# fallenshock/SinDDM

Measured on AMD Instinct MI355X. Metric: diffusion steps/sec (finest scale) + imgs/sec full multi-scale sample, 1/2/4/8 GPU, higher is better.
Workload: dtype f32 (3x3 convs: binary16 hi/lo split products -- Winograd-domain GEMMs with all 4 MFMA terms, fp32 accumulate; fp32-equivalent, error vs float64 = the fp32 oracle's: tests/test_gpu_h2.py; everything else fp32); 1 GPU; C3: 6-scale pyramid, T=1000, finest scale 411x512, batch 64 per GPU, dim=160; batch_per_gpu=64, global_batch=64, scale=5, parallelism=independent chains over 1 GPU(s), one all-gather of the images

## Files before the change

### include/sinddm_hip_debug.h

```cpp
#ifndef SINDDM_HIP_DEBUG_H
#define SINDDM_HIP_DEBUG_H

#include <stddef.h>
#include <stdint.h>

#ifdef __cplusplus
extern "C" {
#endif

int sinddm_prof_begin(void);
int sinddm_prof_end(double* conv_ms_total, int64_t* conv_launches, double* conv_flops_total);
int sinddm_prof_end2(double* conv_ms_total, int64_t* conv_launches, double* conv_flops_total,
                     double* conv_exec_flops_total);
int sinddm_prof_end3(int kind, double* ms_total, int64_t* launches, double* flops_total,
                     double* exec_flops_total, int reset);

int sinddm_debug_conv_path(int dim, int B, int H, int W);

int sinddm_debug_infer_path(int dim, int B, int H, int W);

int sinddm_debug_train_path(int dim, int B, int H, int W);

int sinddm_debug_block_train(const float* params, const float* packed, const float* packed_bwd, int dim, int l,
                             const float* x, const float* cond_bias, const float* grad_y, float* y, float* grad_x,
                             float* grad_params, float* dcond, int B, int H, int W, void* ws, size_t ws_bytes,
                             void* stream);

int sinddm_debug_wgrad_map(int Cin, int Cout, int64_t ntiles, int ncu, uint32_t* wg_out, int wg_cap, int32_t* splits_out,
                           int splits_cap);

#ifdef __cplusplus
}
#endif
#endif
```

### sinddm_amd/_lib.py

```python
from __future__ import annotations

import ctypes as C
import os
from typing import Optional

import torch

_HERE = os.path.dirname(os.path.abspath(__file__))
LIB_PATH = os.path.join(_HERE, "libsinddm_hip.so")

ABI_SYMBOLS = (
    "sinddm_abi_version", "sinddm_param_count", "sinddm_param_tensors", "sinddm_param_offset",
    "sinddm_packed_count", "sinddm_workspace_bytes", "sinddm_pack_weights", "sinddm_net_forward",
    "sinddm_q_sample", "sinddm_reverse_step", "sinddm_reverse_step_edit", "sinddm_upsample_bilinear", "sinddm_prof_begin", "sinddm_prof_end", "sinddm_prof_end2", "sinddm_prof_end3", "sinddm_debug_wgrad_map", "sinddm_debug_conv_path",
    "sinddm_debug_block_train", "sinddm_debug_infer_path", "sinddm_debug_train_path",
    "sinddm_train_workspace_bytes", "sinddm_packed_bwd_count", "sinddm_pack_weights_bwd",
    "sinddm_net_forward_train", "sinddm_net_backward", "sinddm_l1_loss_fwd_bwd", "sinddm_adam_ema_step",
    "sinddm_cond_embed", "sinddm_cond_stride", "sinddm_sample_chain", "sinddm_sample_chain2", "sinddm_sample_chain_ex",
    "sinddm_normal_fill", "sinddm_wrap_halo", "sinddm_upsample_bilinear_wrap", "sinddm_sample_chain_tile",
    "sinddm_sample_chain_keep", "sinddm_reverse_step_keep", "sinddm_normal_fill_samples", "sinddm_sample_chain_seeds",
)


ABI_VERSION = 3
DIM_FP32_CONVS = 0x10000
TILE_HALO = 16


class StepCoefs(C.Structure):
    _fields_ = [("mode", C.c_int), ("clip", C.c_int),
                ("sqrt_recip_ac_t", C.c_float), ("sqrt_recipm1_ac_t", C.c_float),
                ("coef1_t", C.c_float), ("coef2_t", C.c_float),
                ("gamma_t", C.c_float), ("gamma_tm1", C.c_float),
                ("sqrt_ac_tm1", C.c_float), ("sqrt_ac_t", C.c_float), ("sqrt_1m_ac_t", C.c_float),
                ("sqrt_1m_ac_tm1_mvar", C.c_float), ("sigma", C.c_float)]


class ChainOpts(C.Structure):
    _fields_ = [("edit_w", C.c_void_p), ("edit_c", C.c_void_p), ("noise", C.c_void_p)]


class KeepOpts(C.Structure):
    _fields_ = [("mask", C.c_void_p), ("x0", C.c_void_p), ("ab", C.POINTER(C.c_float))]
# ... 45 lines not shown
                                         i, i, i, i, p, sz, p, p, C.POINTER(C.c_int), C.POINTER(ChainOpts), i, i]),
        "sinddm_sample_chain_keep": (i, [p, p, p, p, p, p, C.POINTER(StepCoefs), C.POINTER(C.c_int), i, f, C.c_uint64, C.c_uint64,
                                         i, i, i, i, p, sz, p, p, C.POINTER(C.c_int), C.POINTER(ChainOpts), i, i,
                                         C.POINTER(KeepOpts)]),
        "sinddm_sample_chain_seeds": (i, [p, p, p, p, p, p, C.POINTER(StepCoefs), C.POINTER(C.c_int), i, f, C.c_uint64, C.c_uint64,
                                          i, i, i, i, p, sz, p, p, C.POINTER(C.c_int), C.POINTER(ChainOpts), i, i,
                                          C.POINTER(KeepOpts), p]),
        "sinddm_normal_fill_samples": (i, [p, i, i64, p, C.c_uint64, p]),
        "sinddm_reverse_step_keep": (i, [p, p, p, p, p, C.POINTER(StepCoefs), p, p, p, p, f, f, i, i, i, p]),
        "sinddm_wrap_halo": (i, [p, p, i, i, i, i, i, p]),
        "sinddm_upsample_bilinear_wrap": (i, [p, p, i, i, i, i, i, i, i, p]),
        "sinddm_normal_fill": (i, [p, i64, C.c_uint64, C.c_uint64, p]),
        "sinddm_upsample_bilinear": (i, [p, p, i, i, i, i, i, p]),
        "sinddm_prof_begin": (i, []),
        "sinddm_prof_end": (i, [C.POINTER(C.c_double), C.POINTER(C.c_int64), C.POINTER(C.c_double)]),
        "sinddm_prof_end2": (i, [C.POINTER(C.c_double), C.POINTER(C.c_int64), C.POINTER(C.c_double),
                                 C.POINTER(C.c_double)]),
        "sinddm_prof_end3": (i, [i, C.POINTER(C.c_double), C.POINTER(C.c_int64), C.POINTER(C.c_double),
                                 C.POINTER(C.c_double), i]),
        "sinddm_debug_wgrad_map": (i, [i, i, i64, i, C.POINTER(C.c_uint32), i, C.POINTER(C.c_int32), i]),
        "sinddm_debug_conv_path": (i, [i, i, i, i]),
        "sinddm_debug_infer_path": (i, [i, i, i, i]),
        "sinddm_debug_train_path": (i, [i, i, i, i]),
        "sinddm_debug_block_train": (i, [p, p, p, i, i, p, p, p, p, p, p, p, i, i, i, p, sz, p]),
        "sinddm_train_workspace_bytes": (sz, [i, i, i, i]),
        "sinddm_packed_bwd_count": (i64, [i]),
        "sinddm_pack_weights_bwd": (i, [p, p, i, p]),
        "sinddm_net_forward_train": (i, [p, p, p, p, i, f, p, i, i, i, i, p, sz, p]),
        "sinddm_net_backward": (i, [p, p, p, p, p, p, p, i, i, i, i, p, sz, p]),
        "sinddm_l1_loss_fwd_bwd": (i, [p, p, p, p, i64, f, p]),
        "sinddm_adam_ema_step": (i, [p, p, p, p, p, f, f, f, f, f, f, f, i, i64, p]),
    }
    for name, (res, args) in sig.items():
        if not hasattr(lib, name):
            continue
        fn = getattr(lib, name)
        fn.restype = res
        fn.argtypes = args
    _lib = lib
    return lib


def missing_symbols():
    lib = load()
    return [s for s in ABI_SYMBOLS if not hasattr(lib, s)]

# ... 20 lines not shown
```

### sinddm_amd/csrc/conv1x1.h

```cpp
#pragma once
#include "conv_mfma.h"

namespace sinddm {

constexpr int C1_THREADS = 256;
constexpr int C1_PIX = 256;
constexpr int C1_KC = 16;
constexpr int C1_PS = C1_PIX + 16;

template <int MT>
__global__ __launch_bounds__(C1_THREADS) void conv1x1_mfma_kernel(ConvArgs p, int tiles_per_img) {
    constexpr int CO_LDS = ConvCfg<MT, 4>::CO_LDS;
    constexpr int W_FLOATS = C1_KC * CO_LDS;
    constexpr int BUF = W_FLOATS + C1_KC * C1_PS;
    typedef __attribute__((address_space(3))) void* lds_ptr;
    extern __shared__ __attribute__((aligned(16))) float smem[];

    const int cb = blockIdx.y;
    const int tile = blockIdx.x;
    const int b = tile / tiles_per_img;
    const int p0 = (tile - b * tiles_per_img) * C1_PIX;
    const int tid = threadIdx.x, lane = tid & 63;
    const int wave = __builtin_amdgcn_readfirstlane(tid >> 6);
    const int l16 = lane & 15, kq = lane >> 4;
// ... 235 lines not shown
#pragma unroll
                    for (int j = 0; j < 4; ++j) v[j] = gelu_erf(v[j]);
                } else if constexpr (ACT == 2) {
#pragma unroll
                    for (int j = 0; j < 4; ++j) v[j] *= gelu_erf_grad(uv[mt & 1][r][j]);
                }
                if constexpr (RES) v += rv[mt & 1][r];
                if (C1B_ABL & 4) { if (v[0] + v[1] + v[2] + v[3] == 123.4f) p.out[tid] = v[1]; continue; }
                const unsigned o = off[mt & 1][r];
                __builtin_amdgcn_raw_buffer_store_b128(__builtin_bit_cast(u32x4, v), rs_out, (int)(straddle ? OOB : o), 0, 0);
                if (tail_tile && straddle) {
                    float* q = p.out + samp + (size_t)(co0 + mt * 16 + kq * 4 + r) * HW + px0;
#pragma unroll
                    for (int j = 0; j < 3; ++j)
                        if (j < keep) q[j] = v[j];
                }
            }
        }
        ctx = nctx;
    }
}

template <int MTT>
inline void conv1x1_all_launch(const ConvArgs& a, int tpi, int ntiles, hipStream_t st) {
    const size_t lds = ((size_t)((a.Cin2 + 15) / 16 * 4) * MTT * 64 + MTT * 16) * sizeof(float);
    const int cus = 256;
    const dim3 grid((unsigned)(ntiles < 2 * cus ? ntiles : 2 * cus), (unsigned)(a.Cout / (MTT * 16)));
#define C1B_GO(ACT, RES)                                                                                                \
    do {                                                                                                                \
        if ((a.H * a.W) % 4 == 0)                                                                                       \
            hipLaunchKernelGGL((conv1x1_all_kernel<MTT, ACT, 0, RES>), grid, dim3(C1_THREADS), lds, st, a, tpi, ntiles); \
        else                                                                                                            \
            hipLaunchKernelGGL((conv1x1_all_kernel<MTT, ACT, 1, RES>), grid, dim3(C1_THREADS), lds, st, a, tpi, ntiles); \
    } while (0)
    const int res = a.resid != nullptr;
    switch ((a.act & 0xff) * 2 + res) {
        case 0: C1B_GO(0, 0); break;
        case 1: C1B_GO(0, 1); break;
        case 2: C1B_GO(1, 0); break;
        case 3: C1B_GO(1, 1); break;
        case 4: C1B_GO(2, 0); break;
        default: C1B_GO(2, 1);
    }
#undef C1B_GO
}

#ifndef SINDDM_CONV1X1_V2
#define SINDDM_CONV1X1_V2 1
#endif
#ifndef SINDDM_CONV1X1_TAIL
#define SINDDM_CONV1X1_TAIL 1
#endif

inline int conv1x1_launch(const ConvArgs& a, int mt, hipStream_t st) {
    ConvProfiler& prof = conv_profiler();
    const bool rec = prof.on && prof.used < ConvProfiler::MAXREC;
    if (rec) {
        while (prof.created <= prof.used) {
            (void)hipEventCreate(&prof.ev[2 * prof.created]);
            (void)hipEventCreate(&prof.ev[2 * prof.created + 1]);
            ++prof.created;
        }
        (void)hipEventRecord(prof.ev[2 * prof.used], st);
    }
    const int HW = a.H * a.W;
    const int tpi = (HW + C1_PIX - 1) / C1_PIX;
    const dim3 grid((unsigned)(a.B * tpi), (unsigned)a.coblks);
    const int mtt = mt * a.coblks;
    if (SINDDM_CONV1X1_V2 && mt == 5 && (mtt == 5 || mtt == 10) && a.Cout == mtt * 16 && (SINDDM_CONV1X1_TAIL || HW % 4 == 0) && a.Cin2 <= 160) {
        const int ntiles = a.B * tpi;
        const size_t lds_all = ((size_t)((a.Cin2 + 15) / 16 * 4) * mtt * 64 + mtt * 16) * sizeof(float);
        if (ntiles >= 512 && mtt == 10 && lds_all <= 64 * 1024) conv1x1_all_launch<10>(a, tpi, ntiles, st);
        else if (ntiles >= 128) conv1x1_all_launch<5>(a, tpi, ntiles, st);
        else conv1x1_all_launch<1>(a, tpi, ntiles, st);
    } else
    switch (mt) {
        case 5: { constexpr size_t lds = 2 * (C1_KC * ConvCfg<5, 4>::CO_LDS + C1_KC * C1_PS) * sizeof(float);
                  hipLaunchKernelGGL(conv1x1_mfma_kernel<5>, grid, dim3(C1_THREADS), lds, st, a, tpi); break; }
        case 2: { constexpr size_t lds = 2 * (C1_KC * ConvCfg<2, 4>::CO_LDS + C1_KC * C1_PS) * sizeof(float);
                  hipLaunchKernelGGL(conv1x1_mfma_kernel<2>, grid, dim3(C1_THREADS), lds, st, a, tpi); break; }
        case 1: { constexpr size_t lds = 2 * (C1_KC * ConvCfg<1, 4>::CO_LDS + C1_KC * C1_PS) * sizeof(float);
                  hipLaunchKernelGGL(conv1x1_mfma_kernel<1>, grid, dim3(C1_THREADS), lds, st, a, tpi); break; }
        default: return SINDDM_E_BADSHAPE;
    }
    if (rec) {
        (void)hipEventRecord(prof.ev[2 * prof.used + 1], st);
        const double fl = 2.0 * a.B * a.H * a.W * (double)a.Cout * (double)a.Cin2;
        prof.note(2, fl, fl);
    }
    SINDDM_LAUNCH_CHECK();
    return 0;
}

}
```

### sinddm_amd/csrc/internal.h

```cpp
#pragma once
#include "common.h"

namespace sinddm {

struct PackSeg {
    long long dst;
    long long count;
    long long w;
    long long w2;
    int kind;
    int cin, cout, taps, nch, mt, co_lds;
    int transpose;
};
struct PackArgs {
    PackSeg seg[32];
    int nseg;
    long long total;
};
int pack_launch(const float* params, float* packed, const PackArgs& a, hipStream_t st);

struct TrainBufs {
    float* cond;
    float* emb;
    float* hpre;
    float* cvec;
    float* mvec;
    float* h[4];
    float* u[4];
    float* g[4];
    float* o[4];
    float* s[4];
    float* dcond;
    float* small;
    float* wscr;
    float* amax;
};

struct ChainStep;
int net_forward_impl(const NetPlan& P, const float* params, const float* packed, const float* x, const int64_t* t_dev,
                     int t_host, float scale, float* out, int B, int H, int W, void* ws, size_t ws_bytes,
                     hipStream_t st, const TrainBufs* tb, const ChainStep* cs = nullptr);

int block_forward(const NetPlan& P, int l, const float* params, const float* packed, const float* cur, const float* cond,
                  int cond_stride, float* hbuf, float* gbuf, float* obuf, float* upre, int B, int H, int W, hipStream_t st,
                  int Wt = 0, float* amax = nullptr);
int conv3x3_path(int cout, int cin, int coblks, int B, int H, int W);

struct ConvArgs;
bool wh_applies(const NetPlan& P, int B, int H, int W, int cin, int cout);
bool wh_enabled();
int wh_conv(const ConvArgs& c, hipStream_t st);
int wh_pack(const float* w, float* wsinv, void* img, int cin, int cout, int transpose, hipStream_t st);
int amax_tensor_launch(const float* x, float* amax, int B, long long per_sample, hipStream_t st);

int dwconv_launch(const float* x, const float* w, const float* bias, const float* cond, int cond_stride,
                  const float* addt, int flip, float* out, int B, int C, int H, int W, hipStream_t st, int pi = 0, int po = 0,
                  float* amax = nullptr);

}
```

### sinddm_amd/csrc/sinddm_fwd.hip

```cpp
#include "conv_mfma.h"
#include "conv_wino.h"
#include "conv_wino4.h"
#include "conv_wh.h"
#include "internal.h"
namespace sinddm {

ConvProfiler& conv_profiler() {
    static ConvProfiler p;
    return p;
}

__global__ void pack_kernel(const float* __restrict__ params, float* __restrict__ packed, PackArgs a) {
    long long i = (long long)blockIdx.x * blockDim.x + threadIdx.x;
    if (i >= a.total) return;
    int s = 0;
    long long base = 0;
    while (s < a.nseg - 1 && i >= base + a.seg[s].count) { base += a.seg[s].count; ++s; }
    const PackSeg& g = a.seg[s];
    const long long j = i - base;
    float v = 0.0f;
    if (g.kind == 0) {
        const int co_l = (int)(j % g.co_lds);
        long long r = j / g.co_lds;
        const int kc = (int)(r % KC); r /= KC;
// ... 347 lines not shown
        for (int h = 0; h < 2; ++h) {
            const int gx = x0 + lane + 64 * h;
            if (gx < po) {
#pragma unroll
                for (int r = 0; r < DW_RW; ++r) {
                    const int gy = y0 + wv * DW_RW + r;
                    if (gy < H) {
                        const size_t oidx = plane + (size_t)gy * po + gx;
                        const float ov = gx < W ? (addt ? o[r][h] + addt[oidx] : o[r][h]) : 0.0f;
                        mx = fmaxf(mx, fabsf(ov));
                        out[oidx] = ov;
                    }
                }
            }
        }
    }
    if (amax) amax_publish(mx, amax + (size_t)b * AMAX_STRIDE);
}

#ifndef DWR_ROWS_
#define DWR_ROWS_ 12
#endif
constexpr int DWR_ROWS = DWR_ROWS_;

__global__ __launch_bounds__(256) void dwconv5_rows_kernel(const float* __restrict__ x, const float* __restrict__ w,
                                                            const float* __restrict__ bias, const float* __restrict__ cond,
                                                            int cond_stride, const float* __restrict__ addt, int flip,
                                                            float* __restrict__ out, int C, int H, int W, int bandsX, int Wt,
                                                            float* __restrict__ amax) {
    const int c = blockIdx.y, b = blockIdx.z;
    const int by = blockIdx.x / bandsX, bx = blockIdx.x - by * bandsX;
    const int lane = threadIdx.x & 63, wv = threadIdx.x >> 6;
    const int x4 = (bx * 64 + lane) * 4;
    const int y0 = (by * 4 + wv) * DWR_ROWS;
    const size_t plane = ((size_t)b * C + c) * H * W;
    float wk[25];
#pragma unroll
    for (int k = 0; k < 25; ++k) wk[k] = w[c * 25 + (flip ? 24 - k : k)];
    const float add = (bias ? bias[c] : 0.0f) + (cond ? cond[(size_t)b * cond_stride + c] : 0.0f);
    if (y0 >= H) return;
    const __amdgpu_buffer_rsrc_t rsx = __builtin_amdgcn_make_buffer_rsrc(const_cast<float*>(x + plane), 0, H * W * 4, 0x00020000);
    constexpr int OOBI = 0x40000000;
    const bool colok = x4 < W;
    const bool lok = colok && x4 >= 4, rok = colok && x4 + 4 < W;
    f32x4 acc[DWR_ROWS];
#pragma unroll
    for (int r = 0; r < DWR_ROWS; ++r) acc[r] = f32x4{add, add, add, add};
#pragma unroll
    for (int ir = 0; ir < DWR_ROWS + 4; ++ir) {
        const int gy = y0 + ir - 2;
        const bool rowok = gy >= 0 && gy < H;
        const int base = (gy * W + x4) * 4;
        const f32x4 ql = __builtin_bit_cast(f32x4, __builtin_amdgcn_raw_buffer_load_b128(rsx, (rowok && lok) ? base - 16 : OOBI, 0, 0));
        const f32x4 qm = __builtin_bit_cast(f32x4, __builtin_amdgcn_raw_buffer_load_b128(rsx, (rowok && colok) ? base : OOBI, 0, 0));
        const f32x4 qr = __builtin_bit_cast(f32x4, __builtin_amdgcn_raw_buffer_load_b128(rsx, (rowok && rok) ? base + 16 : OOBI, 0, 0));
        const float in[8] = {ql[2], ql[3], qm[0], qm[1], qm[2], qm[3], qr[0], qr[1]};
#pragma unroll
        for (int r = 0; r < DWR_ROWS; ++r) {
            const int ky = ir - r;
            if (ky >= 0 && ky < 5) {
#pragma unroll
                for (int kx = 0; kx < 5; ++kx) {
#pragma unroll
                    for (int cc = 0; cc < 4; ++cc) acc[r][cc] = fmaf(wk[ky * 5 + kx], in[cc + kx], acc[r][cc]);
                }
            }
        }
    }
    float mx = 0.f;
#pragma unroll
    for (int r = 0; r < DWR_ROWS; ++r) {
        const int gy = y0 + r;
        if (colok && gy < H) {
            const size_t o = plane + (size_t)gy * W + x4;
            f32x4 v = acc[r];
            if (addt) v += *reinterpret_cast<const f32x4*>(addt + o);
            if (x4 + 4 > Wt) {
#pragma unroll
                for (int cc = 0; cc < 4; ++cc) v[cc] = x4 + cc < Wt ? v[cc] : 0.0f;
            }
            mx = fmaxf(fmaxf(mx, fmaxf(fabsf(v[0]), fabsf(v[1]))), fmaxf(fabsf(v[2]), fabsf(v[3])));
            *reinterpret_cast<f32x4*>(out + o) = v;
        }
    }
    if (amax) amax_publish(mx, amax + (size_t)b * AMAX_STRIDE);
}

#ifndef SINDDM_DW_ROWS
#define SINDDM_DW_ROWS 1
#endif

int dwconv_launch(const float* x, const float* w, const float* bias, const float* cond, int cond_stride,
                  const float* addt, int flip, float* out, int B, int C, int H, int W, hipStream_t st, int pi, int po,
                  float* amax) {
    if (pi <= 0) pi = W;
    if (po <= 0) po = W;
    if (SINDDM_DW_ROWS && pi % 4 == 0 && po == pi && pi >= 192) {
        const int bandsX = (pi + 255) / 256, bandsY = (H + 4 * DWR_ROWS - 1) / (4 * DWR_ROWS);
// ... 635 lines not shown
}
static size_t fwd_workspace_core(const NetPlan& P, int B, int H, int W) {
    const size_t act = align_up((size_t)B * P.dim * H * fwd_pitch(P, W) * sizeof(float), 256);
    return cond_region_bytes(P, B) + 4 * act + fwd_xpad_bytes(P, B, H, W);
}
static size_t fwd_workspace_bytes(const NetPlan& P, int B, int H, int W) {
    return fwd_workspace_core(P, B, H, W) + 2 * cond_region_bytes(P, (B + 1) / 2) + 4096;
}

struct ChainStep {
    const float* cond_row;
    const float* x_tilde;
    float* x_next;
    sinddm_step_coefs coefs;
    unsigned long long seed, stream_id;
    int b0;
    const float* edit_w;
    const float* edit_c;
    const float* noise;
    const float* keep_m;
    const float* keep_x0;
    float keep_a, keep_b;
    const unsigned long long* sseeds;
};

#define SINDDM_TAIL_LAUNCH(KERNEL, variant, grid, st, ...)                                                             \
    do {                                                                                                              \
        switch (variant) {                                                                                            \
            case 0: hipLaunchKernelGGL((KERNEL<false, false, false>), grid, dim3(256), 0, st, __VA_ARGS__); break;    \
            case 1: hipLaunchKernelGGL((KERNEL<true, false, false>), grid, dim3(256), 0, st, __VA_ARGS__); break;     \
            case 2: hipLaunchKernelGGL((KERNEL<false, true, false>), grid, dim3(256), 0, st, __VA_ARGS__); break;     \
            case 3: hipLaunchKernelGGL((KERNEL<true, true, false>), grid, dim3(256), 0, st, __VA_ARGS__); break;      \
            case 4: hipLaunchKernelGGL((KERNEL<false, false, true>), grid, dim3(256), 0, st, __VA_ARGS__); break;     \
            case 5: hipLaunchKernelGGL((KERNEL<true, false, true>), grid, dim3(256), 0, st, __VA_ARGS__); break;      \
            case 6: hipLaunchKernelGGL((KERNEL<false, true, true>), grid, dim3(256), 0, st, __VA_ARGS__); break;      \
            default: hipLaunchKernelGGL((KERNEL<true, true, true>), grid, dim3(256), 0, st, __VA_ARGS__); break;      \
        }                                                                                                             \
    } while (0)
static int tail_variant(const float* edit_w, const float* noise, const float* keep_m) {
    return (edit_w ? 1 : 0) | (noise ? 2 : 0) | (keep_m ? 4 : 0);
}

int conv3x3_path(int cout, int cin, int coblks, int B, int H, int W) {
    if (!wino_enabled() || cout % 4 != 0) return 0;
    const bool f24 = mt_for(cout) == 5 && cout % 80 == 0 && cin >= 16 && cin % 16 == 0;
    const bool v3 = SINDDM_WINO_V3 && f24 &&
                    (long long)B * ((W + 31) / 32) * ((H + 3) / 4) * coblks >= SINDDM_V3_MIN_ITEMS_PER_CU * wino2_cu_count();
    if (v3 && SINDDM_WINO_V4 && conv_wino4_applies(B, H, W, coblks)) return 4;
    return v3 ? 3 : 2;
}

int block_forward(const NetPlan& P, int l, const float* params, const float* packed, const float* cur, const float* cond,
                  int cond_stride, float* hbuf, float* gbuf, float* obuf, float* upre, int B, int H, int W, hipStream_t st,
                  int Wt, float* amax) {
    const BlockPlan& b = P.blk[l];
    const bool wha = amax && b.pk_q1 >= 0 && conv_wh_applies(P.fp32_convs, B, H, W, b.cin, b.cout);
    const bool whb = amax && b.pk_q2 >= 0 && conv_wh_applies(P.fp32_convs, B, H, W, b.cout, b.cout);
    int rc = Wt > 0 ? dwconv_launch(cur, params + b.dw_w, params + b.dw_b, cond, cond_stride, nullptr, 0, hbuf, B, b.cin, H,
                                    Wt, st, W, W, wha ? amax : nullptr)
                    : dwconv_launch(cur, params + b.dw_w, params + b.dw_b, cond, cond_stride, nullptr, 0, hbuf, B, b.cin, H,
                                    W, st, 0, 0, wha ? amax : nullptr);
    if (rc) return rc;
    const bool wino = wino_enabled();
    ConvArgs c1{};
    c1.in = hbuf; c1.bias = packed + b.pk_b1; c1.out = gbuf;
    c1.B = B; c1.H = H; c1.W = W; c1.Cin = b.cin; c1.Cout = b.cout; c1.nch1 = 0;
    c1.coblks = b.coblks; c1.act = 1; c1.zero = packed + P.pk_zero; c1.Wt = Wt;
    c1.out_pre = upre;
    constexpr int c3 = SINDDM_CONV_C3;
    const bool v3 = SINDDM_WINO_V3 && wino &&
                    (long long)B * ((W + 31) / 32) * ((H + 3) / 4) * b.coblks >= SINDDM_V3_MIN_ITEMS_PER_CU * wino2_cu_count();
    const bool v4 = SINDDM_WINO_V4 && v3 && conv_wino4_applies(B, H, W, b.coblks);
    if (wha) {
        c1.w3 = packed + b.pk_q1; c1.wsinv = packed + b.pk_qs1; c1.amax_in = amax; c1.amax_out = whb ? amax + 1 : nullptr;
        c1.bias = params + b.c1_b;
        rc = conv_wh_launch(c1, st);
    } else if (v3 && b.pk_w1f >= 0) {
        c1.w3 = packed + b.pk_w1f; c1.nch3 = b.nchw1;
        rc = v4 ? conv_wino4_launch(c1, st) : conv_wino3_launch(c1, st);
    } else if (wino && b.pk_wc1 >= 0 && b.cin % 4 == 0) {
        c1.w3 = packed + b.pk_wc1; c1.nch3 = b.nchw1;
        rc = conv_wino_launch(c1, b.mt, st);
    } else if (b.cin == 3 && c3) {
        const int nwg = ((H * W + 255) / 256) * B;
        int split = 1;
        while (split < 8 && nwg * split < 2048 && b.cout % (split * 2) == 0) split *= 2;
        hipLaunchKernelGGL(conv3x3_c3_gelu_kernel, dim3((H * W + 255) / 256, B, split), dim3(256), 0, st, hbuf,
                           params + b.c1_w, params + b.c1_b, gbuf, c1.out_pre, H, W, b.cout, b.cout / split, Wt > 0 ? Wt : W,
                           whb ? amax + 1 : nullptr);
        SINDDM_LAUNCH_CHECK();
        rc = 0;
    } else {
        c1.w3 = packed + b.pk_c1; c1.nch3 = b.nch1;
        rc = conv_launch(c1, b.mt, st);
    }
    if (rc) return rc;
    if (whb && !(wha || (b.cin == 3 && c3 && !(v3 && b.pk_w1f >= 0) && !(wino && b.pk_wc1 >= 0 && b.cin % 4 == 0)))) {
        rc = amax_tensor_launch(gbuf, amax + 1, B, (long long)b.cout * H * W, st);
        if (rc) return rc;
    }
    ConvArgs c2{};
    c2.in = gbuf; c2.out = obuf;
    c2.B = B; c2.H = H; c2.W = W; c2.Cin = b.cout; c2.Cout = b.cout;
    c2.coblks = b.coblks; c2.act = 0; c2.zero = packed + P.pk_zero; c2.Wt = Wt;
    if (wino && b.cout % 4 == 0) {
        if (b.nchr > 0) {
            ConvArgs r1{};
            r1.in2 = cur; r1.Cin2 = b.cin; r1.w1 = packed + b.pk_res; r1.nch1 = b.nchr; r1.nch3 = 0;
            r1.bias = packed + b.pk_b2; r1.out = obuf; r1.Cout = b.cout; r1.coblks = b.coblks;
            r1.B = B; r1.H = H; r1.W = W; r1.zero = packed + P.pk_zero;
            rc = conv1x1_launch(r1, b.mt, st);
            if (rc) return rc;
            c2.resid = obuf; c2.bias = nullptr;
        } else {
            c2.resid = cur; c2.bias = packed + b.pk_b2;
        }
        c2.nch1 = 0;
        if (whb) {
            c2.w3 = packed + b.pk_q2; c2.wsinv = packed + b.pk_qs2; c2.amax_in = amax + 1;
            rc = conv_wh_launch(c2, st);
        } else if (v3 && b.pk_w2f >= 0) {
            c2.w3 = packed + b.pk_w2f; c2.nch3 = b.nchw2;
            rc = v4 ? conv_wino4_launch(c2, st) : conv_wino3_launch(c2, st);
        } else {
            c2.w3 = packed + b.pk_wc2; c2.nch3 = b.nchw2;
            rc = conv_wino_launch(c2, b.mt, st);
        }
    } else {
        c2.w3 = packed + b.pk_c2; c2.bias = packed + b.pk_b2; c2.nch3 = b.nch2;
        if (b.nchr > 0) { c2.in2 = cur; c2.Cin2 = b.cin; c2.w1 = packed + b.pk_res; c2.nch1 = b.nchr; }
        else { c2.resid = cur; c2.nch1 = 0; }
        rc = conv_launch(c2, b.mt, st);
    }
    return rc;
}
// ... 76 lines not shown
        }
        if (!any) amax = nullptr;
        else if (hipMemsetAsync(amax, 0, (size_t)B * AMAX_STRIDE * sizeof(float), st) != hipSuccess) return SINDDM_E_BADARG;
    }
    const float* cur = x;
    if (padded) {
        const long long nrows = (long long)B * CHANNELS * H;
        const long long nq = nrows * (Wp / 4);
        hipLaunchKernelGGL(pad_rows_kernel, dim3((unsigned)((nq + 255) / 256)), dim3(256), 0, st, x, xpad, H, W, Wp, nrows);
        SINDDM_LAUNCH_CHECK();
        cur = xpad;
    }
    int freeb[4] = {0, 1, 2, 3};
    int curb = -1;
    for (int l = 0; l < 4; ++l) {
        const BlockPlan& b = P.blk[l];
        int sel[3], n = 0;
        for (int i = 0; i < 4 && n < 3; ++i)
            if (freeb[i] != curb) sel[n++] = freeb[i];
        float* hbuf = tb ? tb->h[l] : fb.buf[sel[0]];
        float* gbuf = tb ? tb->g[l] : fb.buf[sel[1]];
        float* obuf = tb ? tb->o[l] : fb.buf[sel[2]];
        const int rc = block_forward(P, l, params, packed, cur, fb.cond + b.cond_off, cond_stride, hbuf, gbuf, obuf,
                                     tb ? tb->u[l] : nullptr, B, H, Wp, st, padded ? W : 0, amax ? amax + 2 * l : nullptr);
        if (rc) return rc;
        cur = obuf;
        curb = sel[2];
    }
    const int HW = H * W;
    if (padded) {
        const unsigned gx = (unsigned)((H * (Wp / 4) + 255) / 256);
        if (cs && cs->x_next)
            SINDDM_TAIL_LAUNCH(final_conv_reverse_step_pitch_kernel, tail_variant(cs->edit_w, cs->noise, cs->keep_m), dim3(gx, B),
                               st, cur, params + P.fin_w, params + P.fin_b, x, cs->x_tilde, cs->x_next, cs->coefs, P.half, H, W,
                               Wp, cs->seed, cs->stream_id, cs->b0, cs->edit_w, cs->edit_c, cs->noise, cs->keep_m, cs->keep_x0,
                               cs->keep_a, cs->keep_b, cs->sseeds);
        else
            hipLaunchKernelGGL(final_conv1x1_pitch_kernel, dim3(gx, B), dim3(256), 0, st, cur, params + P.fin_w,
                               params + P.fin_b, out, P.half, H, W, Wp);
        SINDDM_LAUNCH_CHECK();
        return 0;
    }
    if (cs && cs->x_next && HW % 4 == 0) {
        SINDDM_TAIL_LAUNCH(final_conv_reverse_step_kernel, tail_variant(cs->edit_w, cs->noise, cs->keep_m),
                           dim3((HW / 4 + 255) / 256, B), st, cur, params + P.fin_w, params + P.fin_b, x, cs->x_tilde, cs->x_next,
                           cs->coefs, P.half, HW, cs->seed, cs->stream_id, cs->b0, cs->edit_w, cs->edit_c, cs->noise, cs->keep_m,
                           cs->keep_x0, cs->keep_a, cs->keep_b, cs->sseeds);
// ... 166 lines not shown
    NetPlan p = make_plan(dim);
    if (!p.ok) return SINDDM_E_BADSHAPE;
    hipStream_t st = static_cast<hipStream_t>(stream);
    hipStream_t sx = static_cast<hipStream_t>(aux_stream);
    const long long n = (long long)B * CHANNELS * H * W;
    long long bx = ((n + 3) / 4 + 255) / 256;
    if (bx > 8192) bx = 8192;
    if (ws_bytes < fwd_workspace_bytes(p, B, H, W)) return SINDDM_E_WORKSPACE;
    float* cond_tab = static_cast<float*>(ws);
    const bool fuse_tail = (H * W) % 4 == 0 || fwd_pitch(p, W) != W;
    const long long items = (long long)B * ((fwd_pitch(p, W) + 31) / 32) * ((H + 7) / 8) * 2;
    const long long ncu = wino2_cu_count();
    const long long rounds = (items + ncu - 1) / ncu;
    bool split = sx != nullptr && sx != st && B >= 2 && fuse_tail && n_steps > 0 && items < SINDDM_SPLIT_ITEMS_HI * ncu &&
                 items >= SINDDM_SPLIT_ITEMS_LO * ncu && (rounds * ncu - items) * 25 >= rounds * ncu;
    if (split && conv_wh_applies(p.fp32_convs, B, H, fwd_pitch(p, W), p.dim, p.dim))
        split = false;
    if (split && cond_region_bytes(p, B) + fwd_workspace_core(p, (B + 1) / 2, H, W) + fwd_workspace_core(p, B - (B + 1) / 2, H, W) > ws_bytes)
        split = false;
    const int Bh[2] = {split ? (B + 1) / 2 : B, split ? B - (B + 1) / 2 : 0};
    char* wsh[2] = {static_cast<char*>(ws), nullptr};
    size_t wsz[2] = {ws_bytes, 0};
    hipEvent_t ev_go = nullptr, ev_done = nullptr;
    if (split) {
        wsh[0] = static_cast<char*>(ws) + cond_region_bytes(p, B);
        wsz[0] = fwd_workspace_core(p, Bh[0], H, W);
        wsh[1] = wsh[0] + wsz[0];
        wsz[1] = fwd_workspace_core(p, Bh[1], H, W);
        if (hipEventCreateWithFlags(&ev_go, hipEventDisableTiming) != hipSuccess) return SINDDM_E_BADARG;
        if (hipEventCreateWithFlags(&ev_done, hipEventDisableTiming) != hipSuccess) {
            (void)hipEventDestroy(ev_go);
            return SINDDM_E_BADARG;
        }
    }
    const size_t hoff = (size_t)Bh[0] * CHANNELS * H * W;
    float* cur = x;
    float* nxt = x_alt;
    int rc = 0;
    if (tiled) rc = wrap_halo_launch(x, nullptr, B * CHANNELS, Hc, Wc, halo_y, halo_x, st);
    for (int i0 = 0; i0 < n_steps && rc == 0;) {
        int len = 1, dt = 0;
        if (i0 + 1 < n_steps) {
            dt = t_list[i0 + 1] - t_list[i0];
            len = 2;
            while (i0 + len < n_steps && len < CHAIN_COND_ROWS && t_list[i0 + len] - t_list[i0 + len - 1] == dt) ++len;
        }
// ... 4 lines not shown
        for (int l = 0; l < 4; ++l) {
            ca.mlp_w[l] = p.blk[l].mlp_w; ca.mlp_b[l] = p.blk[l].mlp_b;
            ca.tr_w[l] = p.blk[l].tr_w; ca.tr_b[l] = p.blk[l].tr_b;
            ca.cin[l] = p.blk[l].cin; ca.coff[l] = p.blk[l].cond_off;
        }
        hipLaunchKernelGGL(cond_kernel, dim3(len), dim3(128), 0, st, ca);
        if (hipGetLastError() != hipSuccess) { rc = SINDDM_E_BADARG; break; }
        if (split) {
            if (hipEventRecord(ev_go, st) != hipSuccess || hipStreamWaitEvent(sx, ev_go, 0) != hipSuccess) { rc = SINDDM_E_BADARG; break; }
        }
        for (int i = i0; i < i0 + len && rc == 0; ++i) {
            if (coefs[i].mode != 0 && !x_tilde) { rc = SINDDM_E_BADARG; break; }
            for (int h = 0; h < (split ? 2 : 1) && rc == 0; ++h) {
                const size_t o = h ? hoff : 0;
                ChainStep cs{};
                cs.cond_row = cond_tab + (size_t)(i - i0) * p.cond_stride;
                cs.x_tilde = x_tilde ? x_tilde + o : nullptr; cs.x_next = fuse_tail ? nxt + o : nullptr; cs.coefs = coefs[i];
                cs.seed = (unsigned long long)seed; cs.stream_id = (unsigned long long)(stream_id0 + (uint64_t)i);
                cs.b0 = h ? Bh[0] : 0;
                cs.edit_w = edit_w; cs.edit_c = edit_c; cs.noise = noise ? noise + (size_t)i * (size_t)n : nullptr;
                cs.keep_m = keep_m; cs.keep_x0 = keep_x0;
                if (keep_m) { cs.keep_a = keep_ab[2 * i]; cs.keep_b = keep_ab[2 * i + 1]; }
                cs.sseeds = sseeds ? sseeds + (h ? Bh[0] : 0) : nullptr;
                rc = net_forward_impl(p, params, packed, cur + o, nullptr, t_list[i], scale, eps + o, Bh[h], H, W, wsh[h], wsz[h],
                                      h ? sx : st, nullptr, &cs);
                if (tiled && fuse_tail && rc == 0)
                    rc = wrap_halo_launch(nxt + o, nullptr, Bh[h] * CHANNELS, Hc, Wc, halo_y, halo_x, h ? sx : st);
            }
            if (rc) break;
            if (!fuse_tail && sseeds) {
                const int chw = CHANNELS * H * W;
                unsigned gx = (unsigned)(((chw + 3) / 4 + 255) / 256);
                if (gx > 8192) gx = 8192;
                const unsigned long long sid = (unsigned long long)(stream_id0 + (uint64_t)i);
                const float ka = keep_m ? keep_ab[2 * i] : 1.0f, kb = keep_m ? keep_ab[2 * i + 1] : 0.0f;
#define SINDDM_SEEDED_TAIL(E, K)                                                                                          \
    hipLaunchKernelGGL((reverse_step_rng_samples_kernel<E, K>), dim3(gx, (unsigned)B), dim3(256), 0, st, cur, eps, x_tilde, nxt,  \
                       coefs[i], sid, sseeds, edit_w, edit_c, chw, H * W, keep_m, keep_x0, ka, kb)
                if (edit_w && keep_m) SINDDM_SEEDED_TAIL(true, true);
                else if (edit_w) SINDDM_SEEDED_TAIL(true, false);
                else if (keep_m) SINDDM_SEEDED_TAIL(false, true);
                else SINDDM_SEEDED_TAIL(false, false);
#undef SINDDM_SEEDED_TAIL
                if (hipGetLastError() != hipSuccess) { rc = SINDDM_E_BADARG; break; }
                if (tiled && (rc = wrap_halo_launch(nxt, nullptr, B * CHANNELS, Hc, Wc, halo_y, halo_x, st)) != 0) break;
            } else if (!fuse_tail) {
                SINDDM_TAIL_LAUNCH(reverse_step_rng_kernel, tail_variant(edit_w, noise, keep_m), dim3((unsigned)bx), st, cur, eps,
                                   x_tilde, nxt, coefs[i], n, (unsigned long long)seed,
                                   (unsigned long long)(stream_id0 + (uint64_t)i), edit_w, edit_c,
                                   noise ? noise + (size_t)i * (size_t)n : nullptr, CHANNELS * H * W, H * W, keep_m, keep_x0,
                                   keep_m ? keep_ab[2 * i] : 1.0f, keep_m ? keep_ab[2 * i + 1] : 0.0f);
                if (hipGetLastError() != hipSuccess) { rc = SINDDM_E_BADARG; break; }
                if (tiled && (rc = wrap_halo_launch(nxt, nullptr, B * CHANNELS, Hc, Wc, halo_y, halo_x, st)) != 0) break;
            }
            float* t_ = cur; cur = nxt; nxt = t_;
        }
        if (split) {
            if (hipEventRecord(ev_done, sx) != hipSuccess || hipStreamWaitEvent(st, ev_done, 0) != hipSuccess) {
                (void)hipStreamSynchronize(sx);
                if (!rc) rc = SINDDM_E_BADARG;
            }
        }
        i0 += len;
    }
    if (split) {
        (void)hipEventDestroy(ev_go);
        (void)hipEventDestroy(ev_done);
    }
    if (rc) return rc;
    if (result_in_alt) *result_in_alt = (cur == x_alt) ? 1 : 0;
    return 0;
}

int sinddm_sample_chain_ex(const float* params, const float* packed, float* x, float* x_alt, float* eps, const float* x_tilde,
                           const sinddm_step_coefs* coefs, const int* t_list, int n_steps, float scale, uint64_t seed,
                           uint64_t stream_id0, int dim, int B, int H, int W, void* ws, size_t ws_bytes, void* stream,
                           void* aux_stream, int* result_in_alt, const sinddm_chain_opts* opts) {
    return sample_chain_impl(params, packed, x, x_alt, eps, x_tilde, coefs, t_list, n_steps, scale, seed, stream_id0, dim, B, H, W,
                             ws, ws_bytes, stream, aux_stream, result_in_alt, opts, 0, 0, nullptr, nullptr);
}

int sinddm_sample_chain_tile(const float* params, const float* packed, float* x, float* x_alt, float* eps, const float* x_tilde,
                             const sinddm_step_coefs* coefs, const int* t_list, int n_steps, float scale, uint64_t seed,
                             uint64_t stream_id0, int dim, int B, int H, int W, void* ws, size_t ws_bytes, void* stream,
                             void* aux_stream, int* result_in_alt, const sinddm_chain_opts* opts, int halo_y, int halo_x) {
    return sinddm_sample_chain_keep(params, packed, x, x_alt, eps, x_tilde, coefs, t_list, n_steps, scale, seed, stream_id0, dim, B,
                                    H, W, ws, ws_bytes, stream, aux_stream, result_in_alt, opts, halo_y, halo_x, nullptr);
}

int sinddm_sample_chain_keep(const float* params, const float* packed, float* x, float* x_alt, float* eps, const float* x_tilde,
                             const sinddm_step_coefs* coefs, const int* t_list, int n_steps, float scale, uint64_t seed,
// ... 109 lines not shown
    p.flops = 0.0;
    p.exec_flops = 0.0;
    return 0;
}

int sinddm_prof_end(double* conv_ms_total, int64_t* conv_launches, double* conv_flops_total) {
    return sinddm_prof_end2(conv_ms_total, conv_launches, conv_flops_total, nullptr);
}

int sinddm_prof_end2(double* conv_ms_total, int64_t* conv_launches, double* conv_flops_total,
                     double* conv_exec_flops_total) {
    return sinddm_prof_end3(0, conv_ms_total, conv_launches, conv_flops_total, conv_exec_flops_total, 1);
}

int sinddm_debug_infer_path(int dim, int B, int H, int W) {
    NetPlan p = make_plan(dim);
    if (!p.ok || B <= 0 || H <= 0 || W <= 0) return SINDDM_E_BADARG;
    const BlockPlan& b = p.blk[2];
    const int Wp = fwd_pitch(p, W);
    if (b.pk_q2 >= 0 && conv_wh_applies(p.fp32_convs, B, H, Wp, b.cout, b.cout)) return 8;
    return conv3x3_path(b.cout, b.cout, b.coblks, B, H, Wp);
}

int sinddm_prof_end3(int kind, double* ms_total, int64_t* launches, double* flops_total, double* exec_flops_total,
                     int reset) {
    ConvProfiler& p = conv_profiler();
    p.on = false;
    double ms = 0.0, fl = 0.0, ex = 0.0;
    int64_t n = 0;
    for (int i = 0; i < p.used; ++i) {
        if (kind >= 10 ? (p.kind[i] != kind / 10 || p.gen[i] != kind % 10) : (kind != 0 && p.kind[i] != kind)) continue;
        hipError_t e = hipEventSynchronize(p.ev[2 * i + 1]);
        if (e != hipSuccess) return (int)e;
        float t = 0.f;
        e = hipEventElapsedTime(&t, p.ev[2 * i], p.ev[2 * i + 1]);
        if (e != hipSuccess) return (int)e;
        ms += t; fl += p.rec_flops[i]; ex += p.rec_exec[i]; ++n;
    }
    if (ms_total) *ms_total = ms;
    if (launches) *launches = n;
    if (flops_total) *flops_total = fl;
    if (exec_flops_total) *exec_flops_total = ex;
    if (reset) { p.used = 0; p.flops = 0.0; p.exec_flops = 0.0; }
    return 0;
}

// ... 31 lines not shown
```

Baseline: 721.2 sample-steps/s (finest scale, batch x steps/s, all GPUs).

## Overlap residual 1x1 projection on side stream; prefetch rows in depthwise conv

Each block's residual 1x1 projection now forks onto an auxiliary stream, gated by events, so it runs alongside the depthwise conv and first 3x3 conv on the main stream, using a reduced workgroups-per-CU grid. The 5x5 depthwise row kernel is restructured with a rolling register prefetch of input rows, narrower 64-bit edge loads, packed fp32x2 FMAs and a 4-waves occupancy bound. A debug entry point for the dwconv kernel is also added. The stream fork adds event overhead per block and the concurrent kernels compete for CUs, while the prefetch raises register pressure.

```diff
diff --git a/include/sinddm_hip_debug.h b/include/sinddm_hip_debug.h
--- a/include/sinddm_hip_debug.h
+++ b/include/sinddm_hip_debug.h
@@ -26,6 +26,10 @@
                              float* grad_params, float* dcond, int B, int H, int W, void* ws, size_t ws_bytes,
                              void* stream);
 
+int sinddm_debug_dwconv(const float* x, const float* w, const float* bias, const float* cond, int cond_stride,
+                        const float* addt, int flip, float* out, int B, int C, int H, int W, int Wt, float* amax,
+                        void* stream);
+
 int sinddm_debug_wgrad_map(int Cin, int Cout, int64_t ntiles, int ncu, uint32_t* wg_out, int wg_cap, int32_t* splits_out,
                            int splits_cap);
 
diff --git a/sinddm_amd/_lib.py b/sinddm_amd/_lib.py
--- a/sinddm_amd/_lib.py
+++ b/sinddm_amd/_lib.py
@@ -19,6 +19,7 @@
     "sinddm_cond_embed", "sinddm_cond_stride", "sinddm_sample_chain", "sinddm_sample_chain2", "sinddm_sample_chain_ex",
     "sinddm_normal_fill", "sinddm_wrap_halo", "sinddm_upsample_bilinear_wrap", "sinddm_sample_chain_tile",
     "sinddm_sample_chain_keep", "sinddm_reverse_step_keep", "sinddm_normal_fill_samples", "sinddm_sample_chain_seeds",
+    "sinddm_debug_dwconv",
 )
 
 
@@ -110,6 +111,7 @@
         "sinddm_debug_conv_path": (i, [i, i, i, i]),
         "sinddm_debug_infer_path": (i, [i, i, i, i]),
         "sinddm_debug_train_path": (i, [i, i, i, i]),
+        "sinddm_debug_dwconv": (i, [p, p, p, p, i, p, i, p, i, i, i, i, i, p, p]),
         "sinddm_debug_block_train": (i, [p, p, p, i, i, p, p, p, p, p, p, p, i, i, i, p, sz, p]),
         "sinddm_train_workspace_bytes": (sz, [i, i, i, i]),
         "sinddm_packed_bwd_count": (i64, [i]),
diff --git a/sinddm_amd/csrc/conv1x1.h b/sinddm_amd/csrc/conv1x1.h
--- a/sinddm_amd/csrc/conv1x1.h
+++ b/sinddm_amd/csrc/conv1x1.h
@@ -281,10 +281,10 @@
 }
 
 template <int MTT>
-inline void conv1x1_all_launch(const ConvArgs& a, int tpi, int ntiles, hipStream_t st) {
+inline void conv1x1_all_launch(const ConvArgs& a, int tpi, int ntiles, hipStream_t st, int wg_per_cu) {
     const size_t lds = ((size_t)((a.Cin2 + 15) / 16 * 4) * MTT * 64 + MTT * 16) * sizeof(float);
     const int cus = 256;
-    const dim3 grid((unsigned)(ntiles < 2 * cus ? ntiles : 2 * cus), (unsigned)(a.Cout / (MTT * 16)));
+    const dim3 grid((unsigned)(ntiles < wg_per_cu * cus ? ntiles : wg_per_cu * cus), (unsigned)(a.Cout / (MTT * 16)));
 #define C1B_GO(ACT, RES)                                                                                                \
     do {                                                                                                                \
         if ((a.H * a.W) % 4 == 0)                                                                                       \
@@ -311,7 +311,7 @@
 #define SINDDM_CONV1X1_TAIL 1
 #endif
 
-inline int conv1x1_launch(const ConvArgs& a, int mt, hipStream_t st) {
+inline int conv1x1_launch(const ConvArgs& a, int mt, hipStream_t st, int wg_per_cu = 2) {
     ConvProfiler& prof = conv_profiler();
     const bool rec = prof.on && prof.used < ConvProfiler::MAXREC;
     if (rec) {
@@ -329,9 +329,9 @@
     if (SINDDM_CONV1X1_V2 && mt == 5 && (mtt == 5 || mtt == 10) && a.Cout == mtt * 16 && (SINDDM_CONV1X1_TAIL || HW % 4 == 0) && a.Cin2 <= 160) {
         const int ntiles = a.B * tpi;
         const size_t lds_all = ((size_t)((a.Cin2 + 15) / 16 * 4) * mtt * 64 + mtt * 16) * sizeof(float);
-        if (ntiles >= 512 && mtt == 10 && lds_all <= 64 * 1024) conv1x1_all_launch<10>(a, tpi, ntiles, st);
-        else if (ntiles >= 128) conv1x1_all_launch<5>(a, tpi, ntiles, st);
-        else conv1x1_all_launch<1>(a, tpi, ntiles, st);
+        if (ntiles >= 512 && mtt == 10 && lds_all <= 64 * 1024) conv1x1_all_launch<10>(a, tpi, ntiles, st, wg_per_cu);
+        else if (ntiles >= 128) conv1x1_all_launch<5>(a, tpi, ntiles, st, wg_per_cu);
+        else conv1x1_all_launch<1>(a, tpi, ntiles, st, wg_per_cu);
     } else
     switch (mt) {
         case 5: { constexpr size_t lds = 2 * (C1_KC * ConvCfg<5, 4>::CO_LDS + C1_KC * C1_PS) * sizeof(float);
diff --git a/sinddm_amd/csrc/internal.h b/sinddm_amd/csrc/internal.h
--- a/sinddm_amd/csrc/internal.h
+++ b/sinddm_amd/csrc/internal.h
@@ -37,13 +37,17 @@
 };
 
 struct ChainStep;
+struct SideStream {
+    hipStream_t sx;
+    hipEvent_t ev_fork, ev_join;
+};
 int net_forward_impl(const NetPlan& P, const float* params, const float* packed, const float* x, const int64_t* t_dev,
                      int t_host, float scale, float* out, int B, int H, int W, void* ws, size_t ws_bytes,
                      hipStream_t st, const TrainBufs* tb, const ChainStep* cs = nullptr);
 
 int block_forward(const NetPlan& P, int l, const float* params, const float* packed, const float* cur, const float* cond,
                   int cond_stride, float* hbuf, float* gbuf, float* obuf, float* upre, int B, int H, int W, hipStream_t st,
-                  int Wt = 0, float* amax = nullptr);
+                  int Wt = 0, float* amax = nullptr, const SideStream* side = nullptr);
 int conv3x3_path(int cout, int cin, int coblks, int B, int H, int W);
 
 struct ConvArgs;
diff --git a/sinddm_amd/csrc/sinddm_fwd.hip b/sinddm_amd/csrc/sinddm_fwd.hip
--- a/sinddm_amd/csrc/sinddm_fwd.hip
+++ b/sinddm_amd/csrc/sinddm_fwd.hip
@@ -393,15 +393,19 @@
 #define DWR_ROWS_ 12
 #endif
 constexpr int DWR_ROWS = DWR_ROWS_;
-
-__global__ __launch_bounds__(256) void dwconv5_rows_kernel(const float* __restrict__ x, const float* __restrict__ w,
+#ifndef DWR_PF_
+#define DWR_PF_ 6
+#endif
+constexpr int DWR_PF = DWR_PF_;
+
+__global__ __launch_bounds__(256, 4) void dwconv5_rows_kernel(const float* __restrict__ x, const float* __restrict__ w,
                                                             const float* __restrict__ bias, const float* __restrict__ cond,
                                                             int cond_stride, const float* __restrict__ addt, int flip,
                                                             float* __restrict__ out, int C, int H, int W, int bandsX, int Wt,
                                                             float* __restrict__ amax) {
     const int c = blockIdx.y, b = blockIdx.z;
     const int by = blockIdx.x / bandsX, bx = blockIdx.x - by * bandsX;
-    const int lane = threadIdx.x & 63, wv = threadIdx.x >> 6;
+    const int lane = threadIdx.x & 63, wv = __builtin_amdgcn_readfirstlane(threadIdx.x >> 6);
     const int x4 = (bx * 64 + lane) * 4;
     const int y0 = (by * 4 + wv) * DWR_ROWS;
     const size_t plane = ((size_t)b * C + c) * H * W;
@@ -413,30 +417,49 @@
     const __amdgpu_buffer_rsrc_t rsx = __builtin_amdgcn_make_buffer_rsrc(const_cast<float*>(x + plane), 0, H * W * 4, 0x00020000);
     constexpr int OOBI = 0x40000000;
     const bool colok = x4 < W;
-    const bool lok = colok && x4 >= 4, rok = colok && x4 + 4 < W;
-    f32x4 acc[DWR_ROWS];
-#pragma unroll
-    for (int r = 0; r < DWR_ROWS; ++r) acc[r] = f32x4{add, add, add, add};
+    const unsigned cl = (colok && x4 >= 4) ? x4 * 4 - 8 : OOBI;
+    const unsigned cm = colok ? x4 * 4 : OOBI;
+    const unsigned cr = (colok && x4 + 4 < W) ? x4 * 4 + 16 : OOBI;
+    f32x2 ql[DWR_PF], qr[DWR_PF];
+    f32x4 qm[DWR_PF];
+    auto load_row = [&](int ir) __attribute__((always_inline)) {
+        const int gy = y0 + ir - 2;
+        unsigned ro = (unsigned)gy < (unsigned)H ? (unsigned)(gy * W * 4) : (unsigned)OOBI;
+        asm volatile("" : "+s"(ro));
+        const int s = ir % DWR_PF;
+        ql[s] = __builtin_bit_cast(f32x2, __builtin_amdgcn_raw_buffer_load_b64(rsx, (int)(cl + ro), 0, 0));
+        qm[s] = __builtin_bit_cast(f32x4, __builtin_amdgcn_raw_buffer_load_b128(rsx, (int)(cm + ro), 0, 0));
+        qr[s] = __builtin_bit_cast(f32x2, __builtin_amdgcn_raw_buffer_load_b64(rsx, (int)(cr + ro), 0, 0));
+    };
+#pragma unroll
+    for (int ir = 0; ir < DWR_PF; ++ir) load_row(ir);
+    f32x2 acc[DWR_ROWS][2];
+#pragma unroll
+    for (int r = 0; r < DWR_ROWS; ++r) acc[r][0] = acc[r][1] = f32x2{add, add};
 #pragma unroll
     for (int ir = 0; ir < DWR_ROWS + 4; ++ir) {
-        const int gy = y0 + ir - 2;
-        const bool rowok = gy >= 0 && gy < H;
-        const int base = (gy * W + x4) * 4;
-        const f32x4 ql = __builtin_bit_cast(f32x4, __builtin_amdgcn_raw_buffer_load_b128(rsx, (rowok && lok) ? base - 16 : OOBI, 0, 0));
-        const f32x4 qm = __builtin_bit_cast(f32x4, __builtin_amdgcn_raw_buffer_load_b128(rsx, (rowok && colok) ? base : OOBI, 0, 0));
-        const f32x4 qr = __builtin_bit_cast(f32x4, __builtin_amdgcn_raw_buffer_load_b128(rsx, (rowok && rok) ? base + 16 : OOBI, 0, 0));
-        const float in[8] = {ql[2], ql[3], qm[0], qm[1], qm[2], qm[3], qr[0], qr[1]};
+        const int s = ir % DWR_PF;
+        const f32x2 ev[4] = {ql[s], f32x2{qm[s][0], qm[s][1]}, f32x2{qm[s][2], qm[s][3]}, qr[s]};
+        const f32x2 od[3] = {f32x2{ql[s][1], qm[s][0]}, f32x2{qm[s][1], qm[s][2]}, f32x2{qm[s][3], qr[s][0]}};
 #pragma unroll
         for (int r = 0; r < DWR_ROWS; ++r) {
             const int ky = ir - r;
             if (ky >= 0 && ky < 5) {
 #pragma unroll
                 for (int kx = 0; kx < 5; ++kx) {
-#pragma unroll
-                    for (int cc = 0; cc < 4; ++cc) acc[r][cc] = fmaf(wk[ky * 5 + kx], in[cc + kx], acc[r][cc]);
+                    const float wt = wk[ky * 5 + kx];
+                    const f32x2 w2{wt, wt};
+                    const f32x2 i0 = (kx & 1) ? od[kx >> 1] : ev[kx >> 1];
+                    const f32x2 i1 = (kx & 1) ? od[(kx >> 1) + 1] : ev[(kx >> 1) + 1];
+                    acc[r][0] = __builtin_elementwise_fma(w2, i0, acc[r][0]);
+                    acc[r][1] = __builtin_elementwise_fma(w2, i1, acc[r][1]);
                 }
             }
         }
+#pragma unroll
+        for (int r = 0; r < DWR_ROWS; ++r)
+            if (ir - r >= 0 && ir - r < 5) asm volatile("" : "+v"(acc[r][0]), "+v"(acc[r][1]));
+        if (ir + DWR_PF < DWR_ROWS + 4) load_row(ir + DWR_PF);
     }
     float mx = 0.f;
 #pragma unroll
@@ -444,7 +467,7 @@
         const int gy = y0 + r;
         if (colok && gy < H) {
             const size_t o = plane + (size_t)gy * W + x4;
-            f32x4 v = acc[r];
+            f32x4 v{acc[r][0][0], acc[r][0][1], acc[r][1][0], acc[r][1][1]};
             if (addt) v += *reinterpret_cast<const f32x4*>(addt + o);
             if (x4 + 4 > Wt) {
 #pragma unroll
@@ -1126,6 +1149,7 @@
     const float* keep_x0;
     float keep_a, keep_b;
     const unsigned long long* sseeds;
+    const SideStream* side;
 };
 
 #define SINDDM_TAIL_LAUNCH(KERNEL, variant, grid, st, ...)                                                             \
@@ -1154,12 +1178,20 @@
     return v3 ? 3 : 2;
 }
 
-int block_forward(const NetPlan& P, int l, const float* params, const float* packed, const float* cur, const float* cond,
-                  int cond_stride, float* hbuf, float* gbuf, float* obuf, float* upre, int B, int H, int W, hipStream_t st,
-                  int Wt, float* amax) {
+#ifndef SINDDM_SIDE_STREAM
+#define SINDDM_SIDE_STREAM 1
+#endif
+#ifndef SINDDM_SIDE_FIRST
+#define SINDDM_SIDE_FIRST 1
+#endif
+#ifndef SINDDM_SIDE_WG_PER_CU
+#define SINDDM_SIDE_WG_PER_CU 1
+#endif
+
+static int block_head(const NetPlan& P, int l, const float* params, const float* packed, const float* cur, const float* cond,
+                      int cond_stride, float* hbuf, float* gbuf, float* upre, int B, int H, int W, hipStream_t st, int Wt,
+                      float* amax, bool wha, bool whb) {
     const BlockPlan& b = P.blk[l];
-    const bool wha = amax && b.pk_q1 >= 0 && conv_wh_applies(P.fp32_convs, B, H, W, b.cin, b.cout);
-    const bool whb = amax && b.pk_q2 >= 0 && conv_wh_applies(P.fp32_convs, B, H, W, b.cout, b.cout);
     int rc = Wt > 0 ? dwconv_launch(cur, params + b.dw_w, params + b.dw_b, cond, cond_stride, nullptr, 0, hbuf, B, b.cin, H,
                                     Wt, st, W, W, wha ? amax : nullptr)
                     : dwconv_launch(cur, params + b.dw_w, params + b.dw_b, cond, cond_stride, nullptr, 0, hbuf, B, b.cin, H,
@@ -1203,18 +1235,51 @@
         rc = amax_tensor_launch(gbuf, amax + 1, B, (long long)b.cout * H * W, st);
         if (rc) return rc;
     }
+    return 0;
+}
+
+int block_forward(const NetPlan& P, int l, const float* params, const float* packed, const float* cur, const float* cond,
+                  int cond_stride, float* hbuf, float* gbuf, float* obuf, float* upre, int B, int H, int W, hipStream_t st,
+                  int Wt, float* amax, const SideStream* side) {
+    const BlockPlan& b = P.blk[l];
+    const bool wha = amax && b.pk_q1 >= 0 && conv_wh_applies(P.fp32_convs, B, H, W, b.cin, b.cout);
+    const bool whb = amax && b.pk_q2 >= 0 && conv_wh_applies(P.fp32_convs, B, H, W, b.cout, b.cout);
+    const bool wino = wino_enabled();
+    const bool proj = wino && b.cout % 4 == 0 && b.nchr > 0;
+    auto proj_launch = [&](hipStream_t s, int wg_per_cu) {
+        ConvArgs r1{};
+        r1.in2 = cur; r1.Cin2 = b.cin; r1.w1 = packed + b.pk_res; r1.nch1 = b.nchr; r1.nch3 = 0;
+        r1.bias = packed + b.pk_b2; r1.out = obuf; r1.Cout = b.cout; r1.coblks = b.coblks;
+        r1.B = B; r1.H = H; r1.W = W; r1.zero = packed + P.pk_zero;
+        return conv1x1_launch(r1, b.mt, s, wg_per_cu);
+    };
+    const bool fork = side != nullptr && whb && proj;
+    if (fork && (hipEventRecord(side->ev_fork, st) != hipSuccess || hipStreamWaitEvent(side->sx, side->ev_fork, 0) != hipSuccess))
+        return SINDDM_E_BADARG;
+    int rc = 0;
+    if (fork && SINDDM_SIDE_FIRST) rc = proj_launch(side->sx, SINDDM_SIDE_WG_PER_CU);
+    if (!rc) rc = block_head(P, l, params, packed, cur, cond, cond_stride, hbuf, gbuf, upre, B, H, W, st, Wt, amax, wha, whb);
+    if (fork && !SINDDM_SIDE_FIRST && !rc) rc = proj_launch(side->sx, SINDDM_SIDE_WG_PER_CU);
+    if (fork) {
+        if (hipEventRecord(side->ev_join, side->sx) != hipSuccess || hipStreamWaitEvent(st, side->ev_join, 0) != hipSuccess) {
+            (void)hipStreamSynchronize(side->sx);
+            if (!rc) rc = SINDDM_E_BADARG;
+        }
+    }
+    if (rc) return rc;
+    const bool v3 = SINDDM_WINO_V3 && wino &&
+                    (long long)B * ((W + 31) / 32) * ((H + 3) / 4) * b.coblks >= SINDDM_V3_MIN_ITEMS_PER_CU * wino2_cu_count();
+    const bool v4 = SINDDM_WINO_V4 && v3 && conv_wino4_applies(B, H, W, b.coblks);
     ConvArgs c2{};
     c2.in = gbuf; c2.out = obuf;
     c2.B = B; c2.H = H; c2.W = W; c2.Cin = b.cout; c2.Cout = b.cout;
     c2.coblks = b.coblks; c2.act = 0; c2.zero = packed + P.pk_zero; c2.Wt = Wt;
     if (wino && b.cout % 4 == 0) {
-        if (b.nchr > 0) {
-            ConvArgs r1{};
-            r1.in2 = cur; r1.Cin2 = b.cin; r1.w1 = packed + b.pk_res; r1.nch1 = b.nchr; r1.nch3 = 0;
-            r1.bias = packed + b.pk_b2; r1.out = obuf; r1.Cout = b.cout; r1.coblks = b.coblks;
-            r1.B = B; r1.H = H; r1.W = W; r1.zero = packed + P.pk_zero;
-            rc = conv1x1_launch(r1, b.mt, st);
-            if (rc) return rc;
+        if (proj) {
+            if (!fork) {
+                rc = proj_launch(st, 2);
+                if (rc) return rc;
+            }
             c2.resid = obuf; c2.bias = nullptr;
         } else {
             c2.resid = cur; c2.bias = packed + b.pk_b2;
@@ -1337,7 +1402,8 @@
         float* gbuf = tb ? tb->g[l] : fb.buf[sel[1]];
         float* obuf = tb ? tb->o[l] : fb.buf[sel[2]];
         const int rc = block_forward(P, l, params, packed, cur, fb.cond + b.cond_off, cond_stride, hbuf, gbuf, obuf,
-                                     tb ? tb->u[l] : nullptr, B, H, Wp, st, padded ? W : 0, amax ? amax + 2 * l : nullptr);
+                                     tb ? tb->u[l] : nullptr, B, H, Wp, st, padded ? W : 0, amax ? amax + 2 * l : nullptr,
+                                     cs ? cs->side : nullptr);
         if (rc) return rc;
         cur = obuf;
         curb = sel[2];
@@ -1550,6 +1616,16 @@
     char* wsh[2] = {static_cast<char*>(ws), nullptr};
     size_t wsz[2] = {ws_bytes, 0};
     hipEvent_t ev_go = nullptr, ev_done = nullptr;
+    SideStream side{sx, nullptr, nullptr};
+    const bool side_on = SINDDM_SIDE_STREAM && !split && sx != nullptr && sx != st && n_steps > 0 &&
+                         conv_wh_applies(p.fp32_convs, B, H, fwd_pitch(p, W), p.dim, p.dim);
+    if (side_on) {
+        if (hipEventCreateWithFlags(&side.ev_fork, hipEventDisableTiming) != hipSuccess) return SINDDM_E_BADARG;
+        if (hipEventCreateWithFlags(&side.ev_join, hipEventDisableTiming) != hipSuccess) {
+            (void)hipEventDestroy(side.ev_fork);
+            return SINDDM_E_BADARG;
+        }
+    }
     if (split) {
         wsh[0] = static_cast<char*>(ws) + cond_region_bytes(p, B);
         wsz[0] = fwd_workspace_core(p, Bh[0], H, W);
@@ -1600,6 +1676,7 @@
                 cs.keep_m = keep_m; cs.keep_x0 = keep_x0;
                 if (keep_m) { cs.keep_a = keep_ab[2 * i]; cs.keep_b = keep_ab[2 * i + 1]; }
                 cs.sseeds = sseeds ? sseeds + (h ? Bh[0] : 0) : nullptr;
+                cs.side = side_on ? &side : nullptr;
                 rc = net_forward_impl(p, params, packed, cur + o, nullptr, t_list[i], scale, eps + o, Bh[h], H, W, wsh[h], wsz[h],
                                       h ? sx : st, nullptr, &cs);
                 if (tiled && fuse_tail && rc == 0)
@@ -1645,6 +1722,10 @@
         (void)hipEventDestroy(ev_go);
         (void)hipEventDestroy(ev_done);
     }
+    if (side_on) {
+        (void)hipEventDestroy(side.ev_fork);
+        (void)hipEventDestroy(side.ev_join);
+    }
     if (rc) return rc;
     if (result_in_alt) *result_in_alt = (cur == x_alt) ? 1 : 0;
     return 0;
@@ -1800,6 +1881,15 @@
     return conv3x3_path(b.cout, b.cout, b.coblks, B, H, Wp);
 }
 
+int sinddm_debug_dwconv(const float* x, const float* w, const float* bias, const float* cond, int cond_stride,
+                        const float* addt, int flip, float* out, int B, int C, int H, int W, int Wt, float* amax, void* stream) {
+    if (!x || !w || !out || B <= 0 || C <= 0 || H <= 0 || W <= 0 || Wt < 0 || Wt > W) return SINDDM_E_BADARG;
+    if ((long long)H * W * 4 >= 0x40000000LL) return SINDDM_E_BADSHAPE;
+    hipStream_t st = static_cast<hipStream_t>(stream);
+    if (Wt > 0 && Wt != W) return dwconv_launch(x, w, bias, cond, cond_stride, addt, flip, out, B, C, H, Wt, st, W, W, amax);
+    return dwconv_launch(x, w, bias, cond, cond_stride, addt, flip, out, B, C, H, W, st, 0, 0, amax);
+}
+
 int sinddm_prof_end3(int kind, double* ms_total, int64_t* launches, double* flops_total, double* exec_flops_total,
                      int reset) {
     ConvProfiler& p = conv_profiler();
```

Result: slower. 658.8 sample-steps/s (finest scale, batch x steps/s, all GPUs) (-8.6%).
